# olegroshka/vae-channel-dynamics

Hardware: AMD Instinct MI355X
Metric: images/sec SDXL-VAE train step @256x256 (tracking on) (higher is better)
Workload: dtype f32

## Files before the change

### vae-channel-dynamics_amd/csrc/skinny.hip

```cpp
#include "thin_common.h"
#include "launchers.h"

#ifndef VAE_THIN_F32_MFMA
#define VAE_THIN_F32_MFMA 1
#endif

namespace {

using thin::TP;
using thin::TAPS_MAX;
constexpr int NT = 256;

__device__ __forceinline__ void stage_small(const vae_conv_geom& g, const float* __restrict__ S, int Cs_small, int K, int m0,
                                            int mrows, f32x4* __restrict__ sI) {
  const int hw = g.Ho * g.Wo;
  const size_t sbytes = (size_t)g.B * g.Hs * g.Ws * Cs_small * 4u;
  const auto rsS = VAE_BUF_RSRC(S, sbytes < BUF_MAX ? sbytes : BUF_MAX);
  for (int e = threadIdx.x; e < TP * g.taps; e += NT) {
    const int row = e / g.taps, tap = e - row * g.taps;
    const int m = m0 + row;
    const int b = m / hw, rem = m - b * hw;
    const int y = rem / g.Wo, x = rem - y * g.Wo;
    const int kh = (g.taps == 9) ? tap / 3 : 0, kw = (g.taps == 9) ? tap - kh * 3 : 0;
    int sy = 0, sx = 0;
    const bool ok = (m < mrows) && src_pixel(g, y, x, kh, kw, sy, sx);
    const unsigned base = ok ? (unsigned)(((b * g.Hs + sy) * g.Ws + sx) * Cs_small) * 4u : BUF_OOB;
    f32x4 v = {0.f, 0.f, 0.f, 0.f};
#pragma unroll
    for (int s = 0; s < 4; ++s)
      if (s < K) v[s] = __builtin_bit_cast(float, __builtin_amdgcn_raw_buffer_load_b32(rsS, ok ? base + 4u * s : BUF_OOB, 0, 0));
    sI[e] = v;
  }
}

__global__ __launch_bounds__(NT) void conv_smallk_kernel(vae_igemm_args p) {
  __shared__ f32x4 sI[TP * TAPS_MAX];
  const vae_conv_geom g = p.g;
  const int tid = threadIdx.x, lane = tid & 127, half = tid >> 7;
  const int m0 = blockIdx.x * TP;
  const int n = blockIdx.y * 128 + lane;
  const bool nok = n < p.N;
  stage_small(g, p.A, g.Cs, p.K, m0, p.M, sI);

  float w[TAPS_MAX][4];
#pragma unroll
  for (int t = 0; t < TAPS_MAX; ++t)
#pragma unroll
    for (int s = 0; s < 4; ++s)
      w[t][s] = (nok && t < g.taps && s < p.K) ? p.W[(int64_t)n * p.sn + (int64_t)t * p.st + (int64_t)s * p.sk] : 0.f;
  const float bv = (p.bias && nok) ? p.bias[n] : 0.f;
  const bool cbf = p.out_bf16 != 0;
  const size_t obytes = (size_t)p.M * p.ldc * (cbf ? 2u : 4u);
  const auto rsC = VAE_BUF_RSRC(p.C, obytes);
  __syncthreads();

  float tsum = 0.f;
#pragma unroll 4
  for (int i = 0; i < TP / 2; ++i) {
    const int row = half + 2 * i;
    float acc = bv;
#pragma unroll
    for (int t = 0; t < TAPS_MAX; ++t) {
      if (t < g.taps) {
        const f32x4 v = sI[row * g.taps + t];
#pragma unroll
        for (int s = 0; s < 4; ++s) acc += v[s] * w[t][s];
      }
    }
    const int m = m0 + row;
    const bool ok = nok && m < p.M;
    buf_store1_elem(rsC, cbf, ok ? m * p.ldc + n : -1, acc);
    const float stored = cbf ? (float)(__bf16)acc : acc;
    tsum += ok ? fabsf(stored) : 0.f;
  }
  if (p.track) {
    __syncthreads();
    float* red = reinterpret_cast<float*>(sI);
    red[tid] = tsum;
    __syncthreads();
    if (half == 0 && nok) p.track[(int64_t)blockIdx.x * p.N + n] = red[lane] + red[128 + lane];
  }
}

#if VAE_THIN_F32_MFMA
constexpr int WM_LDT = TP + 4;
constexpr int WM_ROWS = 48;
constexpr int WM_ITEMS = (TP * TAPS_MAX + NT - 1) / NT;
constexpr int WG_SI = WM_ROWS * WM_LDT / 4;
static_assert(WG_SI >= TP * TAPS_MAX + 32 && WG_SI >= NT, "LDS of wgrad_smallk_kernel");

template <bool SMALL_X, int XF>
__device__ __forceinline__ bool wgrad_mfma_serves(const vae_wgrad_args& p, const vae_conv_geom& gs) {
  const int wide = SMALL_X ? p.M : p.N, ldv = SMALL_X ? p.ldy : p.g.Cs;
  const bool vbf = (SMALL_X ? p.y_bf16 : p.x_bf16) != 0;
  const uintptr_t v = reinterpret_cast<uintptr_t>(SMALL_X ? p.dY : p.X);
  return gs.taps == TAPS_MAX && wide >= 64 && wide % 2 == 0 && ldv % 2 == 0 && (v & (vbf ? 3u : 7u)) == 0 &&
         (XF == VAE_XF_NONE || (gs.Ho * gs.Wo) % TP == 0);
}

template <bool SMALL_X, int XF>
__device__ __forceinline__ void wgrad_smallk_mfma(const vae_wgrad_args& p, const vae_conv_geom& gs, int ntiles, float* __restrict__ sT) {
  const int tid = threadIdx.x, lane = tid & 63, wave = tid >> 6;
  const int lc = lane & 15, lg = lane >> 4;
  const int split = blockIdx.x;
  const int wide = SMALL_X ? p.M : p.N, narrow = SMALL_X ? p.N : p.M;
  const int cq = blockIdx.y * 128 + wave * 32 + lc * 2;
  const float* __restrict__ V = SMALL_X ? p.dY : p.X;
  const float* __restrict__ S = SMALL_X ? p.X : p.dY;
  const int ldv = SMALL_X ? p.ldy : p.g.Cs, lds_ = SMALL_X ? p.g.Cs : p.ldy;
  const int npixv = gs.B * gs.Ho * gs.Wo, hwv = gs.Ho * gs.Wo;
  const bool vbf = (SMALL_X ? p.y_bf16 : p.x_bf16) != 0;
  const unsigned esV = vbf ? 2u : 4u;
  const size_t vbytes = (size_t)npixv * ldv * esV;
  const auto rsV = VAE_BUF_RSRC(V, vbytes < BUF_MAX ? vbytes : BUF_MAX);
  const auto rsS = thin::narrow_rsrc(S, gs, lds_);

  for (int i = tid; i < (WM_ROWS - 36) * WM_LDT; i += NT) sT[36 * WM_LDT + i] = (SMALL_X && i < WM_LDT) ? 1.f : 0.f;

  f32x4 acc[3][2];
#pragma unroll
  for (int mb = 0; mb < 3; ++mb)
#pragma unroll
    for (int e = 0; e < 2; ++e) acc[mb][e] = f32x4{0.f, 0.f, 0.f, 0.f};
  f32x4 ssum = {0.f, 0.f, 0.f, 0.f};
  float sc[2] = {0.f, 0.f}, sh[2] = {0.f, 0.f};
  int xb = -1;

  auto load_v = [&](uint2 (&rv)[8], int mb_) {
#pragma unroll
    for (int k = 0; k < 8; ++k) {
      const int m = mb_ + 16 * (k >> 2) + (k & 3);
      const int eoff = neg_unless(m < npixv && cq < wide, m * ldv + cq);
      rv[k] = __builtin_bit_cast(uint2, __builtin_amdgcn_raw_buffer_load_b64(rsV, eoff >= 0 ? (unsigned)eoff * esV : BUF_OOB, 0, 0));
    }
  };
  const int trow = tid & (TP - 1), thalf = __builtin_amdgcn_readfirstlane(tid >> 7);
  f32x4 rt[WM_ITEMS];
  auto load_t = [&](int tile, bool valid) {
    int m = tile * TP + trow;
    asm volatile("" : "+v"(m));
#pragma unroll
    for (int i = 0; i < WM_ITEMS; ++i) {
      const int tap = 2 * i + thalf;
      rt[i] = thin::gather4(gs, rsS, lds_, narrow, hwv, m, tap, valid && tap < TAPS_MAX && m < npixv);
    }
  };
  auto store_t = [&]() {
#pragma unroll
    for (int i = 0; i < WM_ITEMS; ++i) {
      const int tap = 2 * i + thalf;
      if (tap < TAPS_MAX) {
#pragma unroll
        for (int s = 0; s < 4; ++s) sT[(tap * 4 + s) * WM_LDT + trow] = rt[i][s];
        if (!SMALL_X && tap == TAPS_MAX / 2) ssum += rt[i];
      }
    }
  };
  auto chunk = [&](const uint2 (&rv)[8], int c) {
#pragma unroll
    for (int h = 0; h < 2; ++h) {
      f32x4 fa[3];
#pragma unroll
      for (int mb = 0; mb < 3; ++mb) fa[mb] = *reinterpret_cast<const f32x4*>(&sT[(mb * 16 + lc) * WM_LDT + c * 32 + h * 16 + 4 * lg]);
#pragma unroll
      for (int j = 0; j < 4; ++j) {
        const uint2 r = rv[h * 4 + j];
        float v[2];
        v[0] = __builtin_bit_cast(float, vbf ? r.x << 16 : r.x);
        v[1] = __builtin_bit_cast(float, vbf ? r.x & 0xffff0000u : r.y);
        if (XF != VAE_XF_NONE) {
#pragma unroll
          for (int e = 0; e < 2; ++e) v[e] = thin::xform1<XF>(v[e], sc[e], sh[e], cq + e < wide);
        }
#pragma unroll
        for (int mb = 0; mb < 3; ++mb)
#pragma unroll
          for (int e = 0; e < 2; ++e) acc[mb][e] = __builtin_amdgcn_mfma_f32_16x16x4f32(fa[mb][j], v[e], acc[mb][e], 0, 0, 0);
      }
    }
  };

  const thin::TileRange tr = thin::tile_range(split, thin::tiles_per_part(ntiles, p.nsplit), ntiles);
  const int pofs = 4 * lg;
  uint2 rva[8], rvb[8];
  if (tr.beg < tr.end) {
    load_t(tr.beg, true);
    load_v(rva, tr.beg * TP + pofs);
  }
  for (int tile = tr.beg; tile < tr.end; ++tile) {
    int mb0 = tile * TP + pofs;
    asm volatile("" : "+v"(mb0));
    const bool more = tile + 1 < tr.end;
    __syncthreads();
    store_t();
    __syncthreads();
    load_t(tile + 1, more);
    if (XF != VAE_XF_NONE) {
      const int b = (tile * TP) / hwv;
      if (b != xb) {
        xb = b;
#pragma unroll
        for (int e = 0; e < 2; ++e) {
          sc[e] = (cq + e < wide) ? p.scale[(int64_t)b * p.g.Cs + cq + e] : 0.f;
          sh[e] = (cq + e < wide) ? p.shift[(int64_t)b * p.g.Cs + cq + e] : 0.f;
        }
      }
    }
    load_v(rvb, mb0 + 32);
    chunk(rva, 0);
    load_v(rva, mb0 + 64);
    chunk(rvb, 1);
    load_v(rvb, mb0 + 96);
    chunk(rva, 2);
    load_v(rva, more ? mb0 + TP : npixv);
    chunk(rvb, 3);
  }

  const thin::Slab sl = thin::slab_of(p, split, TAPS_MAX);
#pragma unroll
  for (int mb = 0; mb < 3; ++mb)
#pragma unroll
    for (int e = 0; e < 2; ++e)
#pragma unroll
      for (int r = 0; r < 4; ++r) {
        const int t = mb * 4 + lg, ch = cq + e;
        if (ch < wide) {
          if (t < TAPS_MAX && r < narrow) thin::slab_store<SMALL_X>(sl, ch, t, r, acc[mb][e][r]);
          if (SMALL_X && mb == 2 && r == 0 && lg == 1 && p.bias_partial) thin::bias_partial_row(p, split)[ch] = acc[mb][e][r];
        }
      }
  if (!SMALL_X && p.bias_partial && blockIdx.y == 0) {
    __syncthreads();
#pragma unroll
    for (int s = 0; s < 4; ++s) sT[s * NT + tid] = ssum[s];
    __syncthreads();
    if (tid < p.M) {
      float t = 0.f;
      for (int i = 0; i < NT; ++i) t += sT[tid * NT + i];
      thin::bias_partial_row(p, split)[tid] = t;
    }
  }
}
#define WG_BOUNDS __launch_bounds__(NT, 4)
#else
constexpr int WG_SI = TP * TAPS_MAX + 32;
#define WG_BOUNDS __launch_bounds__(NT)
#endif

template <bool SMALL_X, int XF>
__global__ WG_BOUNDS void wgrad_smallk_kernel(vae_wgrad_args p, vae_conv_geom gs, int ntiles) {
  __shared__ f32x4 sI[WG_SI];
#if VAE_THIN_F32_MFMA
  if (wgrad_mfma_serves<SMALL_X, XF>(p, gs)) {
    wgrad_smallk_mfma<SMALL_X, XF>(p, gs, ntiles, reinterpret_cast<float*>(sI));
    return;
  }
#endif
  const int tid = threadIdx.x, lane = tid & 127, half = tid >> 7;
  const int split = blockIdx.x;
  const int ch = blockIdx.y * 128 + lane;
  const int wide = SMALL_X ? p.M : p.N, narrow = SMALL_X ? p.N : p.M;
  const bool chok = ch < wide;
  const float* __restrict__ V = SMALL_X ? p.dY : p.X;
  const float* __restrict__ S = SMALL_X ? p.X : p.dY;
  const int ldv = SMALL_X ? p.ldy : p.g.Cs, lds_ = SMALL_X ? p.g.Cs : p.ldy;
  const int npixv = gs.B * gs.Ho * gs.Wo;
  const int hwv = gs.Ho * gs.Wo;
  const bool vbf = (SMALL_X ? p.y_bf16 : p.x_bf16) != 0;
  const size_t vbytes = (size_t)npixv * ldv * (vbf ? 2u : 4u);
  const auto rsV = VAE_BUF_RSRC(V, vbytes < BUF_MAX ? vbytes : BUF_MAX);

  float acc[TAPS_MAX][4];
#pragma unroll
  for (int t = 0; t < TAPS_MAX; ++t)
#pragma unroll
    for (int s = 0; s < 4; ++s) acc[t][s] = 0.f;
  float vsum = 0.f;
  f32x4 ssum = {0.f, 0.f, 0.f, 0.f};
  int xb = -1;
  float xsc = 1.f, xsh = 0.f;

  const thin::TileRange tr = thin::tile_range(split, thin::tiles_per_part(ntiles, p.nsplit), ntiles);
  for (int tile = tr.beg; tile < tr.end; ++tile) {
    const int m0 = tile * TP;
    __syncthreads();
    stage_small(gs, S, lds_, narrow, m0, npixv, sI);
    __syncthreads();
#pragma unroll 4
    for (int i = 0; i < TP / 2; ++i) {
      const int row = half + 2 * i;
      const int m = m0 + row;
      const bool ok = chok && m < npixv;
      float v = buf_load1_elem(rsV, vbf, ok ? m * ldv + ch : -1);
      if (XF != VAE_XF_NONE) {
        const int b = min(m, npixv - 1) / hwv;
        if (b != xb) {
          xb = b;
          xsc = chok ? p.scale[(int64_t)b * p.g.Cs + ch] : 0.f;
          xsh = chok ? p.shift[(int64_t)b * p.g.Cs + ch] : 0.f;
        }
        v = thin::xform1<XF>(v, xsc, xsh, ok);
      }
      if (SMALL_X) vsum += v;
#pragma unroll
      for (int t = 0; t < TAPS_MAX; ++t) {
        if (t < gs.taps) {
          const f32x4 sv = sI[row * gs.taps + t];
#pragma unroll
          for (int s = 0; s < 4; ++s) acc[t][s] += v * sv[s];
          if (!SMALL_X && t == gs.taps / 2) ssum += sv;
        }
      }
    }
  }

  __syncthreads();
  float* red = reinterpret_cast<float*>(sI);
  if (half == 1) {
#pragma unroll
    for (int t = 0; t < TAPS_MAX; ++t)
#pragma unroll
      for (int s = 0; s < 4; ++s) red[lane * 36 + t * 4 + s] = acc[t][s];
    if (SMALL_X) red[128 * 36 + lane] = vsum;
    else if (lane == 0) {
#pragma unroll
      for (int s = 0; s < 4; ++s) red[128 * 36 + s] = ssum[s];
    }
  }
  __syncthreads();
  if (half == 0) {
    const thin::Slab sl = thin::slab_of(p, split, gs.taps);
    if (chok) {
#pragma unroll
      for (int t = 0; t < TAPS_MAX; ++t)
#pragma unroll
        for (int s = 0; s < 4; ++s)
          if (t < gs.taps && s < narrow) thin::slab_store<SMALL_X>(sl, ch, t, s, acc[t][s] + red[lane * 36 + t * 4 + s]);
    }
    if (p.bias_partial) {
      if (SMALL_X) {
        if (chok) thin::bias_partial_row(p, split)[ch] = vsum + red[128 * 36 + lane];
      } else if (blockIdx.y == 0 && lane < p.M) {
        thin::bias_partial_row(p, split)[lane] = ssum[lane] + red[128 * 36 + lane];
      }
    }
  }
}

}

bool conv_smallk_eligible(const vae_igemm_args& a) {
  const vae_conv_geom& g = a.g;
  return a.K <= 4 && a.batch == 1 && a.xf == VAE_XF_NONE && a.res == nullptr && a.alpha == 1.0f && g.taps <= TAPS_MAX &&
         g.mode != VAE_MODE_DGRAD_S2 && thin::desc_fits((size_t)a.M * a.ldc, 4u) && thin::narrow_fits(g);
}
int launch_conv_smallk(const vae_igemm_args& a, hipStream_t st) {
  dim3 grid((unsigned)((a.M + TP - 1) / TP), (unsigned)((a.N + 127) / 128));
  hipLaunchKernelGGL(conv_smallk_kernel, grid, dim3(NT), 0, st, a);
  return 0;
}

int wgrad_smallk_kind(const vae_wgrad_args& a) { return thin::wgrad_kind(a); }
int wgrad_smallk_tiles(const vae_wgrad_args& a) { return thin::wgrad_tiles(a); }

int launch_wgrad_smallk(const vae_wgrad_args& a, hipStream_t st) {
  const int kind = thin::wgrad_kind(a), ntiles = thin::wgrad_tiles(a);
  const vae_conv_geom gs = thin::wgrad_geom(a, kind);
  const dim3 grid = thin::wgrad_grid(a, kind);
  if (kind == 1) hipLaunchKernelGGL((wgrad_smallk_kernel<true, VAE_XF_NONE>), grid, dim3(NT), 0, st, a, gs, ntiles);
  else dispatch_xf_or_silu(a.xf, [&](auto xf) { hipLaunchKernelGGL((wgrad_smallk_kernel<false, decltype(xf)::value>), grid, dim3(NT), 0, st, a, gs, ntiles); });
  return 0;
}

namespace {

constexpr int NTH = thin::TH, NTW = thin::TW, NHW = thin::HW, NHP = thin::HP;
constexpr int NBK = 32, NLD = NBK + 4, NNT = 128;
constexpr int NHQ = NHP * (NBK / 4), NHI = (NHQ + NNT - 1) / NNT;

template <int XF>
__global__ __launch_bounds__(NNT) void conv_smalln_kernel(vae_igemm_args p, int tiles_x, int tiles_y) {
  __shared__ __attribute__((aligned(16))) float sH[NHP * NLD];
  const vae_conv_geom g = p.g;
  const int tid = threadIdx.x;
  const thin::Tile tl = thin::decode(blockIdx.x, tiles_x, tiles_y);
  const int b = tl.b, y0 = tl.y0, x0 = tl.x0;
  const int pr = tid >> 5, px = tid & 31;
  const bool abf = p.a_bf16 != 0;
  const unsigned esA = abf ? 2u : 4u;
  const auto rsA = VAE_BUF_RSRC(reinterpret_cast<const char*>(p.A) + (int64_t)b * g.Hs * g.Ws * g.Cs * esA, (size_t)g.Hs * g.Ws * g.Cs * esA);
  const float* __restrict__ W = p.W;

  float acc[4] = {0.f, 0.f, 0.f, 0.f};
  const int hk4 = tid & 7;
  uint4 rh[NHI];
  int hmask = 0;
  f32x4 rsc = {0.f, 0.f, 0.f, 0.f}, rsh = {0.f, 0.f, 0.f, 0.f};
  auto load_halo = [&](int c0) {
    hmask = 0;
    const int c = c0 + hk4 * 4;
    if (XF != VAE_XF_NONE) {
      const int cs = min(c, p.K - 4);
      rsc = *reinterpret_cast<const f32x4*>(p.scale + (int64_t)b * g.Cs + cs);
      rsh = *reinterpret_cast<const f32x4*>(p.shift + (int64_t)b * g.Cs + cs);
    }
#pragma unroll
    for (int i = 0; i < NHI; ++i) {
      const int q = tid + NNT * i;
      const int pp = q >> 3;
      const int ir = pp / NHW, jc = pp - ir * NHW;
      const int hy = y0 - 1 + ir, hx = x0 - 1 + jc;
      const bool ok = (q < NHQ) && ((unsigned)hy < (unsigned)g.Hs) && ((unsigned)hx < (unsigned)g.Ws) && (c < p.K);
      rh[i] = buf_load4_raw(rsA, esA, ok ? ((hy * g.Ws + hx) * g.Cs + c) : -1);
      hmask |= (ok ? 1 : 0) << i;
    }
  };
  auto store_halo = [&]() {
#pragma unroll
    for (int i = 0; i < NHI; ++i) {
      const int q = tid + NNT * i;
      if (q < NHQ) {
        f32x4 v = raw4_to_f32(rh[i], abf);
#pragma unroll
        for (int e = 0; e < 4; ++e) v[e] = thin::xform1<XF>(v[e], rsc[e], rsh[e], (hmask >> i) & 1);
        *reinterpret_cast<f32x4*>(&sH[(q >> 3) * NLD + hk4 * 4]) = v;
      }
    }
  };

  const int kchunks = (p.K + NBK - 1) / NBK;
  load_halo(0);
  for (int cch = 0; cch < kchunks; ++cch) {
    const int c0 = cch * NBK;
    __syncthreads();
    store_halo();
    __syncthreads();
    if (cch + 1 < kchunks) load_halo(c0 + NBK);
#pragma unroll
    for (int tap = 0; tap < 9; ++tap) {
      const int kh = tap / 3, kw = tap - kh * 3;
      const float* hrow = &sH[((pr + kh) * NHW + px + kw) * NLD];
#pragma unroll
      for (int q = 0; q < NBK / 4; ++q) {
        const f32x4 a = *reinterpret_cast<const f32x4*>(hrow + q * 4);
#pragma unroll
        for (int s = 0; s < 4; ++s) {
          if (s < p.N) {
            const f32x4 w4 = *reinterpret_cast<const f32x4*>(W + (int64_t)s * p.sn + (int64_t)tap * p.st + c0 + q * 4);
#pragma unroll
            for (int e = 0; e < 4; ++e) acc[s] = __builtin_fmaf(a[e], w4[e], acc[s]);
          }
        }
      }
    }
  }

  const int oy = y0 + pr, ox = x0 + px;
  const auto rsC = VAE_BUF_RSRC(p.C + (int64_t)b * g.Ho * g.Wo * p.ldc, (size_t)g.Ho * g.Wo * p.ldc * 4u);
#pragma unroll
  for (int s = 0; s < 4; ++s)
    if (s < p.N) {
      const float v = acc[s] + (p.bias ? p.bias[s] : 0.f);
      __builtin_amdgcn_raw_buffer_store_b32(__builtin_bit_cast(unsigned, v), rsC,
                                            (oy < g.Ho && ox < g.Wo) ? (unsigned)((oy * g.Wo + ox) * p.ldc + s) * 4u : BUF_OOB, 0, 0);
    }
}

}

bool conv_smalln_eligible(const vae_igemm_args& a) {
  const vae_conv_geom& g = a.g;
  return a.N <= 4 && a.K >= NBK && a.K % NBK == 0 && a.sn % 4 == 0 && a.st % 4 == 0 && aligned16(a.W) && a.batch == 1 && a.res == nullptr && a.track == nullptr && a.alpha == 1.0f &&
         a.A16 == nullptr && thin::fwd_same_3x3(g) && g.Wo % NTW == 0 && g.Ho % NTH == 0 && a.sk == 1 && g.Cs % 4 == 0 && aligned16(a.A) &&
         (a.xf == VAE_XF_NONE || (aligned16(a.scale) && aligned16(a.shift))) &&
         thin::desc_fits(thin::image_elems(g), 4u) && thin::desc_fits((size_t)g.Ho * g.Wo * a.ldc, 4u);
}
int launch_conv_smalln(const vae_igemm_args& a, hipStream_t st) {
  int tx, ty;
  const dim3 grid = thin::tile_grid(a.g, tx, ty);
  dispatch_xf_or_silu(a.xf, [&](auto xf) { hipLaunchKernelGGL((conv_smalln_kernel<decltype(xf)::value>), grid, dim3(NNT), 0, st, a, tx, ty); });
  return 0;
}
```

Before: 121.0.

## Add f32 MFMA paths for small-K and small-N thin convolutions

Adds matrix-core (MFMA 16x16x4 f32) code paths for the small-K convolution (the RGB input conv) and the small-N convolution (the output conv), each selected at runtime when its shape conditions hold. The small-K path becomes a persistent-style kernel that processes several tiles per workgroup and prefetches the next tile's gather into registers, which amortizes weight loads. The small-N path computes per-tap partial products for the halo with MFMA, then sums the 9 taps from shared memory. These replace scalar FMA loops but add more shared memory, register pressure and a larger block size for the small-N kernel.

```diff
diff --git a/vae-channel-dynamics_amd/csrc/skinny.hip b/vae-channel-dynamics_amd/csrc/skinny.hip
--- a/vae-channel-dynamics_amd/csrc/skinny.hip
+++ b/vae-channel-dynamics_amd/csrc/skinny.hip
@@ -33,8 +33,124 @@
   }
 }
 
-__global__ __launch_bounds__(NT) void conv_smallk_kernel(vae_igemm_args p) {
+#if VAE_THIN_F32_MFMA
+constexpr int CM_ITEMS = (TP * TAPS_MAX + NT - 1) / NT;
+typedef unsigned int u32x2 __attribute__((ext_vector_type(2)));
+
+__host__ __device__ __forceinline__ bool conv_mfma_serves(const vae_igemm_args& p) {
+  return p.g.taps == TAPS_MAX && p.N >= 64 && p.N % 4 == 0 && p.ldc % 4 == 0 &&
+         (reinterpret_cast<uintptr_t>(p.C) & (p.out_bf16 ? 7u : 15u)) == 0;
+}
+inline int conv_mfma_tiles_per_wg(int ntiles) { return std::max(1, std::min(8, ntiles / 1024)); }
+
+__device__ __forceinline__ void conv_smallk_mfma(const vae_igemm_args& p, f32x4* __restrict__ sI) {
+  const vae_conv_geom g = p.g;
+  const int tid = threadIdx.x, lane = tid & 63, wave = tid >> 6;
+  const int lc = lane & 15, lg = lane >> 4;
+  const int nw = blockIdx.y * 128 + wave * 32;
+  const int hw = g.Ho * g.Wo;
+  const auto rsS = thin::narrow_rsrc(p.A, g, g.Cs);
+  const bool cbf = p.out_bf16 != 0;
+  const unsigned esC = cbf ? 2u : 4u;
+  const auto rsC = VAE_BUF_RSRC(p.C, (size_t)p.M * p.ldc * esC);
+
+  float wa[2][TAPS_MAX];
+  f32x4 bv[2];
+#pragma unroll
+  for (int cb = 0; cb < 2; ++cb) {
+    const int na = nw + cb * 16 + lc, nd = nw + cb * 16 + 4 * lg;
+#pragma unroll
+    for (int t = 0; t < TAPS_MAX; ++t)
+      wa[cb][t] = (na < p.N && lg < p.K) ? p.W[(int64_t)na * p.sn + (int64_t)t * p.st + (int64_t)lg * p.sk] : 0.f;
+#pragma unroll
+    for (int r = 0; r < 4; ++r) bv[cb][r] = (p.bias && nd < p.N) ? p.bias[nd + r] : 0.f;
+  }
+
+  f32x4 rt[CM_ITEMS];
+  auto gather = [&](int tile, bool valid) {
+    const int m0 = tile * TP;
+#pragma unroll
+    for (int i = 0; i < CM_ITEMS; ++i) {
+      const int e = tid + NT * i;
+      const int row = e / TAPS_MAX, tap = e - row * TAPS_MAX;
+      rt[i] = thin::gather4(g, rsS, g.Cs, p.K, hw, m0 + row, tap, valid && e < TP * TAPS_MAX && m0 + row < p.M);
+    }
+  };
+
+  const int ntiles = (p.M + TP - 1) / TP;
+  const thin::TileRange tr = thin::tile_range(blockIdx.x, thin::tiles_per_part(ntiles, (int)gridDim.x), ntiles);
+  const float* __restrict__ sT = reinterpret_cast<const float*>(sI);
+  if (tr.beg < tr.end) gather(tr.beg, true);
+  for (int tile = tr.beg; tile < tr.end; ++tile) {
+    __syncthreads();
+#pragma unroll
+    for (int i = 0; i < CM_ITEMS; ++i) {
+      const int e = tid + NT * i;
+      if (e < TP * TAPS_MAX) sI[e] = rt[i];
+    }
+    __syncthreads();
+    gather(tile + 1, tile + 1 < tr.end);
+
+    f32x4 tsum[2] = {{0.f, 0.f, 0.f, 0.f}, {0.f, 0.f, 0.f, 0.f}};
+#pragma unroll 2
+    for (int pb = 0; pb < TP / 16; ++pb) {
+      const int prow = pb * 16 + lc;
+      f32x4 acc[2] = {bv[0], bv[1]};
+#pragma unroll
+      for (int t = 0; t < TAPS_MAX; ++t) {
+        const float b = sT[(prow * TAPS_MAX + t) * 4 + lg];
+#pragma unroll
+        for (int cb = 0; cb < 2; ++cb) acc[cb] = __builtin_amdgcn_mfma_f32_16x16x4f32(wa[cb][t], b, acc[cb], 0, 0, 0);
+      }
+      const int m = tile * TP + prow;
+#pragma unroll
+      for (int cb = 0; cb < 2; ++cb) {
+        const int nd = nw + cb * 16 + 4 * lg;
+        const bool ok = m < p.M && nd < p.N;
+        const int eoff = neg_unless(ok, m * p.ldc + nd);
+        const unsigned off = eoff >= 0 ? (unsigned)eoff * esC : BUF_OOB;
+        f32x4 stored = acc[cb];
+        if (cbf) {
+          const uint2 h = pack4(acc[cb]);
+          __builtin_amdgcn_raw_buffer_store_b64(u32x2{h.x, h.y}, rsC, off, 0, 0);
+          stored = unpack4(h);
+        } else {
+          __builtin_amdgcn_raw_buffer_store_b128(__builtin_bit_cast(u32x4, acc[cb]), rsC, off, 0, 0);
+        }
+#pragma unroll
+        for (int r = 0; r < 4; ++r) tsum[cb][r] += ok ? fabsf(stored[r]) : 0.f;
+      }
+    }
+    if (p.track) {
+#pragma unroll
+      for (int cb = 0; cb < 2; ++cb) {
+        const int nd = nw + cb * 16 + 4 * lg;
+#pragma unroll
+        for (int r = 0; r < 4; ++r) {
+          float v = tsum[cb][r];
+          v += lane_plus<8>(v);
+          v += lane_plus<4>(v);
+          v += lane_plus<2>(v);
+          v += lane_plus<1>(v);
+          if (lc == 0 && nd < p.N) p.track[(int64_t)tile * p.N + nd + r] = v;
+        }
+      }
+    }
+  }
+}
+#define CK_BOUNDS __launch_bounds__(NT, 4)
+#else
+#define CK_BOUNDS __launch_bounds__(NT)
+#endif
+
+__global__ CK_BOUNDS void conv_smallk_kernel(vae_igemm_args p) {
   __shared__ f32x4 sI[TP * TAPS_MAX];
+#if VAE_THIN_F32_MFMA
+  if (conv_mfma_serves(p)) {
+    conv_smallk_mfma(p, sI);
+    return;
+  }
+#endif
   const vae_conv_geom g = p.g;
   const int tid = threadIdx.x, lane = tid & 127, half = tid >> 7;
   const int m0 = blockIdx.x * TP;
@@ -355,6 +471,14 @@
          g.mode != VAE_MODE_DGRAD_S2 && thin::desc_fits((size_t)a.M * a.ldc, 4u) && thin::narrow_fits(g);
 }
 int launch_conv_smallk(const vae_igemm_args& a, hipStream_t st) {
+#if VAE_THIN_F32_MFMA
+  if (conv_mfma_serves(a)) {
+    const int ntiles = (a.M + TP - 1) / TP;
+    dim3 grid((unsigned)thin::tiles_per_part(ntiles, conv_mfma_tiles_per_wg(ntiles)), (unsigned)((a.N + 127) / 128));
+    hipLaunchKernelGGL(conv_smallk_kernel, grid, dim3(NT), 0, st, a);
+    return 0;
+  }
+#endif
   dim3 grid((unsigned)((a.M + TP - 1) / TP), (unsigned)((a.N + 127) / 128));
   hipLaunchKernelGGL(conv_smallk_kernel, grid, dim3(NT), 0, st, a);
   return 0;
@@ -378,9 +502,145 @@
 constexpr int NBK = 32, NLD = NBK + 4, NNT = 128;
 constexpr int NHQ = NHP * (NBK / 4), NHI = (NHQ + NNT - 1) / NNT;
 
+#if VAE_THIN_F32_MFMA
+constexpr int NM_NT = 256, NM_KMAX = 128;
+constexpr int NM_LDW = NM_KMAX + 4;
+constexpr int NM_ROWS = 9 * 4;
+constexpr int NM_CB = (NHP + 15) / 16;
+constexpr int NM_LDP = NM_CB * 16 + 4;
+constexpr int NM_LDS = NM_ROWS * NM_LDW + NM_ROWS * NM_LDP;
+constexpr int NSH = NM_LDS > NHP * NLD ? NM_LDS : NHP * NLD;
+
+__host__ __device__ __forceinline__ bool smalln_mfma_serves(const vae_igemm_args& p) { return p.K <= NM_KMAX; }
+
 template <int XF>
-__global__ __launch_bounds__(NNT) void conv_smalln_kernel(vae_igemm_args p, int tiles_x, int tiles_y) {
-  __shared__ __attribute__((aligned(16))) float sH[NHP * NLD];
+__device__ __forceinline__ void conv_smalln_mfma(const vae_igemm_args& p, int tiles_x, int tiles_y, float* __restrict__ sM) {
+  float* __restrict__ sW = sM;
+  float* __restrict__ sP = sM + NM_ROWS * NM_LDW;
+  const vae_conv_geom g = p.g;
+  const int tid = threadIdx.x, lane = tid & 63, wave = tid >> 6;
+  const int lc = lane & 15, lg = lane >> 4;
+  const thin::Tile tl = thin::decode(blockIdx.x, tiles_x, tiles_y);
+  const int b = tl.b, y0 = tl.y0, x0 = tl.x0;
+  const bool abf = p.a_bf16 != 0;
+  const unsigned esA = abf ? 2u : 4u;
+  const auto rsA = VAE_BUF_RSRC(reinterpret_cast<const char*>(p.A) + (int64_t)b * g.Hs * g.Ws * g.Cs * esA, (size_t)g.Hs * g.Ws * g.Cs * esA);
+  const int rows = 9 * p.N, rbn = (rows + 15) >> 4;
+  const int k4 = p.K >> 2;
+
+  for (int i = tid; i < NM_ROWS * k4; i += NM_NT) {
+    const int r = i / k4, c4 = i - r * k4;
+    const int tap = r / p.N, s = r - tap * p.N;
+    f32x4 w = {0.f, 0.f, 0.f, 0.f};
+    if (r < rows) w = *reinterpret_cast<const f32x4*>(p.W + (int64_t)s * p.sn + (int64_t)tap * p.st + c4 * 4);
+    *reinterpret_cast<f32x4*>(&sW[r * NM_LDW + c4 * 4]) = w;
+  }
+
+  int eo[4];
+#pragma unroll
+  for (int ci = 0; ci < 4; ++ci) {
+    const int q = (wave + 4 * ci) * 16 + lc;
+    const int ir = q / NHW, jc = q - ir * NHW;
+    const int hy = y0 - 1 + ir, hx = x0 - 1 + jc;
+    const bool ok = (q < NHP) && ((unsigned)hy < (unsigned)g.Hs) && ((unsigned)hx < (unsigned)g.Ws);
+    eo[ci] = neg_unless(ok, (hy * g.Ws + hx) * g.Cs);
+  }
+  const int ncb = wave == 0 ? 4 : 3;
+
+  f32x4 acc[4][3];
+#pragma unroll
+  for (int ci = 0; ci < 4; ++ci)
+#pragma unroll
+    for (int rb = 0; rb < 3; ++rb) acc[ci][rb] = f32x4{0.f, 0.f, 0.f, 0.f};
+
+  uint4 rx[2][4];
+  auto load_x = [&](int c0) {
+#pragma unroll
+    for (int j = 0; j < 2; ++j)
+#pragma unroll
+      for (int ci = 0; ci < 4; ++ci) rx[j][ci] = buf_load4_raw(rsA, esA, (eo[ci] >= 0 && ci < ncb) ? eo[ci] + c0 + 16 * j + 4 * lg : -1);
+  };
+  load_x(0);
+  __syncthreads();
+
+  for (int c0 = 0; c0 < p.K; c0 += NBK) {
+    uint4 cx[2][4];
+#pragma unroll
+    for (int j = 0; j < 2; ++j)
+#pragma unroll
+      for (int ci = 0; ci < 4; ++ci) cx[j][ci] = rx[j][ci];
+    f32x4 sc[2], sh[2];
+#pragma unroll
+    for (int j = 0; j < 2; ++j) {
+      sc[j] = sh[j] = f32x4{0.f, 0.f, 0.f, 0.f};
+      if (XF != VAE_XF_NONE) {
+        sc[j] = *reinterpret_cast<const f32x4*>(p.scale + (int64_t)b * g.Cs + c0 + 16 * j + 4 * lg);
+        sh[j] = *reinterpret_cast<const f32x4*>(p.shift + (int64_t)b * g.Cs + c0 + 16 * j + 4 * lg);
+      }
+    }
+    if (c0 + NBK < p.K) load_x(c0 + NBK);
+#pragma unroll
+    for (int j = 0; j < 2; ++j) {
+      f32x4 fa[3];
+#pragma unroll
+      for (int rb = 0; rb < 3; ++rb) fa[rb] = *reinterpret_cast<const f32x4*>(&sW[min(rb * 16 + lc, NM_ROWS - 1) * NM_LDW + c0 + 16 * j + 4 * lg]);
+#pragma unroll
+      for (int ci = 0; ci < 4; ++ci) {
+        if (ci < ncb) {
+          f32x4 v = raw4_to_f32(cx[j][ci], abf);
+#pragma unroll
+          for (int e = 0; e < 4; ++e) v[e] = thin::xform1<XF>(v[e], sc[j][e], sh[j][e], eo[ci] >= 0);
+#pragma unroll
+          for (int e = 0; e < 4; ++e)
+#pragma unroll
+            for (int rb = 0; rb < 3; ++rb)
+              if (rb < rbn) acc[ci][rb] = __builtin_amdgcn_mfma_f32_16x16x4f32(fa[rb][e], v[e], acc[ci][rb], 0, 0, 0);
+        }
+      }
+    }
+  }
+
+#pragma unroll
+  for (int ci = 0; ci < 4; ++ci)
+#pragma unroll
+    for (int rb = 0; rb < 3; ++rb)
+#pragma unroll
+      for (int r = 0; r < 4; ++r) {
+        const int row = rb * 16 + 4 * lg + r;
+        if (ci < ncb && row < rows) sP[row * NM_LDP + (wave + 4 * ci) * 16 + lc] = acc[ci][rb][r];
+      }
+  __syncthreads();
+
+  if (tid < NTH * NTW) {
+    const int pr = tid >> 5, px = tid & 31;
+    const int oy = y0 + pr, ox = x0 + px;
+    const auto rsC = VAE_BUF_RSRC(p.C + (int64_t)b * g.Ho * g.Wo * p.ldc, (size_t)g.Ho * g.Wo * p.ldc * 4u);
+#pragma unroll
+    for (int s = 0; s < 4; ++s)
+      if (s < p.N) {
+        float y = p.bias ? p.bias[s] : 0.f;
+#pragma unroll
+        for (int tap = 0; tap < 9; ++tap) y += sP[(tap * p.N + s) * NM_LDP + (pr + tap / 3) * NHW + px + tap % 3];
+        __builtin_amdgcn_raw_buffer_store_b32(__builtin_bit_cast(unsigned, y), rsC,
+                                              (oy < g.Ho && ox < g.Wo) ? (unsigned)((oy * g.Wo + ox) * p.ldc + s) * 4u : BUF_OOB, 0, 0);
+      }
+  }
+}
+#define CN_BOUNDS __launch_bounds__(NM_NT)
+#else
+constexpr int NSH = NHP * NLD;
+#define CN_BOUNDS __launch_bounds__(NNT)
+#endif
+
+template <int XF>
+__global__ CN_BOUNDS void conv_smalln_kernel(vae_igemm_args p, int tiles_x, int tiles_y) {
+  __shared__ __attribute__((aligned(16))) float sH[NSH];
+#if VAE_THIN_F32_MFMA
+  if (smalln_mfma_serves(p)) {
+    conv_smalln_mfma<XF>(p, tiles_x, tiles_y, sH);
+    return;
+  }
+#endif
   const vae_conv_geom g = p.g;
   const int tid = threadIdx.x;
   const thin::Tile tl = thin::decode(blockIdx.x, tiles_x, tiles_y);
@@ -478,6 +738,11 @@
 int launch_conv_smalln(const vae_igemm_args& a, hipStream_t st) {
   int tx, ty;
   const dim3 grid = thin::tile_grid(a.g, tx, ty);
-  dispatch_xf_or_silu(a.xf, [&](auto xf) { hipLaunchKernelGGL((conv_smalln_kernel<decltype(xf)::value>), grid, dim3(NNT), 0, st, a, tx, ty); });
+#if VAE_THIN_F32_MFMA
+  const int nt = smalln_mfma_serves(a) ? NM_NT : NNT;
+#else
+  const int nt = NNT;
+#endif
+  dispatch_xf_or_silu(a.xf, [&](auto xf) { hipLaunchKernelGGL((conv_smalln_kernel<decltype(xf)::value>), grid, dim3(nt), 0, st, a, tx, ty); });
   return 0;
 }
```

New measurement: 121.1 (median of 2 runs). About the same (+0.0%).

## Route small-K and small-N 3x3 convs through f32 MFMA kernels

Applied to the files above, without the earlier changes.

Adds an MFMA f32 16x16x4 path for the small-K (input-channel) conv kernel. It stages the im2col tile in LDS and computes 32 output channels per wave with vectorised stores and a shuffle-based tracking reduction. It also rewrites the small-N conv kernel as a 256-thread MFMA GEMM over halo pixels by 9*N tap-channel columns, double-buffering the halo and weights, then sums taps from LDS. This replaces scalar FMA loops with matrix-core work, at the cost of more LDS, a changed block size and wasted MFMA work on padded columns.

```diff
diff --git a/vae-channel-dynamics_amd/csrc/skinny.hip b/vae-channel-dynamics_amd/csrc/skinny.hip
--- a/vae-channel-dynamics_amd/csrc/skinny.hip
+++ b/vae-channel-dynamics_amd/csrc/skinny.hip
@@ -33,8 +33,130 @@
   }
 }
 
+#if VAE_THIN_F32_MFMA
+constexpr int WM_LDT = TP + 4;
+constexpr int WM_ROWS = 48;
+constexpr int WM_ITEMS = (TP * TAPS_MAX + NT - 1) / NT;
+__device__ __forceinline__ void t_gather(f32x4 (&rt)[WM_ITEMS], const vae_conv_geom& gs, __amdgpu_buffer_rsrc_t rsS, int lds_, int narrow,
+                                         int hwv, int npixv, int m, int thalf, bool valid) {
+#pragma unroll
+  for (int i = 0; i < WM_ITEMS; ++i) {
+    const int tap = 2 * i + thalf;
+    rt[i] = thin::gather4(gs, rsS, lds_, narrow, hwv, m, tap, valid && tap < TAPS_MAX && m < npixv);
+  }
+}
+__device__ __forceinline__ void t_store(const f32x4 (&rt)[WM_ITEMS], float* __restrict__ sT, int trow, int thalf) {
+#pragma unroll
+  for (int i = 0; i < WM_ITEMS; ++i) {
+    const int tap = 2 * i + thalf;
+    if (tap < TAPS_MAX) {
+#pragma unroll
+      for (int s = 0; s < 4; ++s) sT[(tap * 4 + s) * WM_LDT + trow] = rt[i][s];
+    }
+  }
+}
+
+__device__ __forceinline__ bool conv_mfma_serves(const vae_igemm_args& p) {
+  const bool cbf = p.out_bf16 != 0;
+  return p.g.taps == TAPS_MAX && p.g.stride == 1 && p.N >= 64 && p.N % 4 == 0 && p.ldc % 4 == 0 &&
+         (reinterpret_cast<uintptr_t>(p.C) & (cbf ? 7u : 15u)) == 0;
+}
+
+__device__ __forceinline__ void conv_smallk_mfma(const vae_igemm_args& p, float* __restrict__ sT) {
+  const vae_conv_geom& g = p.g;
+  const int tid = threadIdx.x, lane = tid & 63, wave = tid >> 6;
+  const int lc = lane & 15, lg = lane >> 4;
+  const int m0 = blockIdx.x * TP;
+  const int nb = blockIdx.y * 128 + wave * 32;
+
+  f32x4 rt[WM_ITEMS];
+  t_gather(rt, g, thin::narrow_rsrc(p.A, g, g.Cs), g.Cs, p.K, g.Ho * g.Wo, p.M, m0 + (tid & (TP - 1)), __builtin_amdgcn_readfirstlane(tid >> 7), true);
+
+  float a[TAPS_MAX][2];
+  f32x4 bv[2];
+#pragma unroll
+  for (int e = 0; e < 2; ++e) {
+    const int n = nb + 16 * e + lc;
+#pragma unroll
+    for (int t = 0; t < TAPS_MAX; ++t) a[t][e] = (n < p.N && lg < p.K) ? p.W[(int64_t)n * p.sn + (int64_t)t * p.st + (int64_t)lg * p.sk] : 0.f;
+#pragma unroll
+    for (int r = 0; r < 4; ++r) {
+      const int nr = nb + 16 * e + 4 * lg + r;
+      bv[e][r] = (p.bias && nr < p.N) ? p.bias[nr] : 0.f;
+    }
+  }
+  const bool cbf = p.out_bf16 != 0;
+  const unsigned esC = cbf ? 2u : 4u;
+  const auto rsC = VAE_BUF_RSRC(p.C, (size_t)p.M * p.ldc * esC);
+
+  t_store(rt, sT, tid & (TP - 1), __builtin_amdgcn_readfirstlane(tid >> 7));
+  __syncthreads();
+
+  f32x4 tsum[2] = {f32x4{0.f, 0.f, 0.f, 0.f}, f32x4{0.f, 0.f, 0.f, 0.f}};
+#pragma unroll
+  for (int c = 0; c < TP / 64; ++c) {
+    f32x4 acc[4][2];
+#pragma unroll
+    for (int q = 0; q < 4; ++q)
+#pragma unroll
+      for (int e = 0; e < 2; ++e) acc[q][e] = bv[e];
+#pragma unroll
+    for (int t = 0; t < TAPS_MAX; ++t) {
+      const f32x4 b = *reinterpret_cast<const f32x4*>(&sT[(t * 4 + lg) * WM_LDT + c * 64 + 4 * lc]);
+#pragma unroll
+      for (int q = 0; q < 4; ++q)
+#pragma unroll
+        for (int e = 0; e < 2; ++e) acc[q][e] = __builtin_amdgcn_mfma_f32_16x16x4f32(a[t][e], b[q], acc[q][e], 0, 0, 0);
+    }
+#pragma unroll
+    for (int q = 0; q < 4; ++q) {
+      const int m = m0 + c * 64 + 4 * lc + q;
+#pragma unroll
+      for (int e = 0; e < 2; ++e) {
+        const int n = nb + 16 * e + 4 * lg;
+        const bool ok = m < p.M && n < p.N;
+        const unsigned off = oob_unless(ok, (unsigned)(m * p.ldc + n) * esC);
+        f32x4 stored = acc[q][e];
+        if (cbf) {
+          const uint2 h = pack4(stored);
+          typedef unsigned int u32x2 __attribute__((ext_vector_type(2)));
+          __builtin_amdgcn_raw_buffer_store_b64(__builtin_bit_cast(u32x2, h), rsC, off, 0, 0);
+          stored = unpack4(h);
+        } else {
+          __builtin_amdgcn_raw_buffer_store_b128(__builtin_bit_cast(u32x4, stored), rsC, off, 0, 0);
+        }
+#pragma unroll
+        for (int r = 0; r < 4; ++r) tsum[e][r] += ok ? fabsf(stored[r]) : 0.f;
+      }
+    }
+  }
+  if (p.track) {
+#pragma unroll
+    for (int e = 0; e < 2; ++e)
+#pragma unroll
+      for (int r = 0; r < 4; ++r) {
+        float v = tsum[e][r];
+#pragma unroll
+        for (int d = 1; d < 16; d *= 2) v += __shfl_xor(v, d, 64);
+        const int n = nb + 16 * e + 4 * lg + r;
+        if (lc == 0 && n < p.N) p.track[(int64_t)blockIdx.x * p.N + n] = v;
+      }
+  }
+}
+constexpr int SK_SI = TAPS_MAX * 4 * WM_LDT / 4;
+#else
+constexpr int SK_SI = TP * TAPS_MAX;
+#endif
+static_assert(SK_SI >= TP * TAPS_MAX, "LDS of conv_smallk_kernel");
+
 __global__ __launch_bounds__(NT) void conv_smallk_kernel(vae_igemm_args p) {
-  __shared__ f32x4 sI[TP * TAPS_MAX];
+  __shared__ f32x4 sI[SK_SI];
+#if VAE_THIN_F32_MFMA
+  if (conv_mfma_serves(p)) {
+    conv_smallk_mfma(p, reinterpret_cast<float*>(sI));
+    return;
+  }
+#endif
   const vae_conv_geom g = p.g;
   const int tid = threadIdx.x, lane = tid & 127, half = tid >> 7;
   const int m0 = blockIdx.x * TP;
@@ -83,9 +205,6 @@
 }
 
 #if VAE_THIN_F32_MFMA
-constexpr int WM_LDT = TP + 4;
-constexpr int WM_ROWS = 48;
-constexpr int WM_ITEMS = (TP * TAPS_MAX + NT - 1) / NT;
 constexpr int WG_SI = WM_ROWS * WM_LDT / 4;
 static_assert(WG_SI >= TP * TAPS_MAX + 32 && WG_SI >= NT, "LDS of wgrad_smallk_kernel");
 
@@ -139,11 +258,7 @@
   auto load_t = [&](int tile, bool valid) {
     int m = tile * TP + trow;
     asm volatile("" : "+v"(m));
-#pragma unroll
-    for (int i = 0; i < WM_ITEMS; ++i) {
-      const int tap = 2 * i + thalf;
-      rt[i] = thin::gather4(gs, rsS, lds_, narrow, hwv, m, tap, valid && tap < TAPS_MAX && m < npixv);
-    }
+    t_gather(rt, gs, rsS, lds_, narrow, hwv, npixv, m, thalf, valid);
   };
   auto store_t = [&]() {
 #pragma unroll
@@ -375,8 +490,169 @@
 namespace {
 
 constexpr int NTH = thin::TH, NTW = thin::TW, NHW = thin::HW, NHP = thin::HP;
-constexpr int NBK = 32, NLD = NBK + 4, NNT = 128;
-constexpr int NHQ = NHP * (NBK / 4), NHI = (NHQ + NNT - 1) / NNT;
+constexpr int NBK = 32, NLD = NBK + 4;
+constexpr int NHQ = NHP * (NBK / 4);
+
+#if VAE_THIN_F32_MFMA
+template <int XF, int NTHR>
+struct HaloStage {
+  static constexpr int NI = (NHQ + NTHR - 1) / NTHR;
+  uint4 rh[NI];
+  int hmask = 0;
+  f32x4 rsc = {0.f, 0.f, 0.f, 0.f}, rsh = {0.f, 0.f, 0.f, 0.f};
+  __device__ __forceinline__ void load(const vae_igemm_args& p, __amdgpu_buffer_rsrc_t rsA, unsigned esA, int b, int y0, int x0, int c0) {
+    const vae_conv_geom& g = p.g;
+    const int tid = threadIdx.x;
+    hmask = 0;
+    const int c = c0 + (tid & 7) * 4;
+    if (XF != VAE_XF_NONE) {
+      const int cs = min(c, p.K - 4);
+      rsc = *reinterpret_cast<const f32x4*>(p.scale + (int64_t)b * g.Cs + cs);
+      rsh = *reinterpret_cast<const f32x4*>(p.shift + (int64_t)b * g.Cs + cs);
+    }
+#pragma unroll
+    for (int i = 0; i < NI; ++i) {
+      const int q = tid + NTHR * i;
+      const int pp = q >> 3;
+      const int ir = pp / NHW, jc = pp - ir * NHW;
+      const int hy = y0 - 1 + ir, hx = x0 - 1 + jc;
+      const bool ok = (q < NHQ) && ((unsigned)hy < (unsigned)g.Hs) && ((unsigned)hx < (unsigned)g.Ws) && (c < p.K);
+      rh[i] = buf_load4_raw(rsA, esA, ok ? ((hy * g.Ws + hx) * g.Cs + c) : -1);
+      hmask |= (ok ? 1 : 0) << i;
+    }
+  }
+  __device__ __forceinline__ void store(float* __restrict__ sH, bool abf) const {
+    const int tid = threadIdx.x;
+#pragma unroll
+    for (int i = 0; i < NI; ++i) {
+      const int q = tid + NTHR * i;
+      if (q < NHQ) {
+        f32x4 v = raw4_to_f32(rh[i], abf);
+#pragma unroll
+        for (int e = 0; e < 4; ++e) v[e] = thin::xform1<XF>(v[e], rsc[e], rsh[e], (hmask >> i) & 1);
+        *reinterpret_cast<f32x4*>(&sH[(q >> 3) * NLD + (tid & 7) * 4]) = v;
+      }
+    }
+  }
+};
+
+constexpr int NNT = 256;
+constexpr int NMB = (NHP + 15) / 16, NHR = NMB * 16;
+constexpr int NLP = NHR + 4;
+constexpr int NWF = 2 * 3 * 64;
+constexpr int NSM = NHR * NLD + NWF * 4;
+static_assert(NSM >= 36 * NLP, "P lies over the halo and the weights");
+
+template <int XF, int NB>
+__device__ __forceinline__ void conv_smalln_mfma(const vae_igemm_args& p, int tiles_x, int tiles_y, float* __restrict__ sH) {
+  constexpr int NIT = NMB * NB, IPW = (NIT + 3) / 4;
+  constexpr int NWI = (2 * NB * 64 + NNT - 1) / NNT;
+  f32x4* __restrict__ sW = reinterpret_cast<f32x4*>(sH + NHR * NLD);
+  const vae_conv_geom& g = p.g;
+  const int tid = threadIdx.x, lane = tid & 63, wave = __builtin_amdgcn_readfirstlane(tid >> 6);
+  const int lc = lane & 15, lg = lane >> 4;
+  const thin::Tile tl = thin::decode(blockIdx.x, tiles_x, tiles_y);
+  const int b = tl.b, y0 = tl.y0, x0 = tl.x0;
+  const bool abf = p.a_bf16 != 0;
+  const unsigned esA = abf ? 2u : 4u;
+  const auto rsA = VAE_BUF_RSRC(reinterpret_cast<const char*>(p.A) + (int64_t)b * g.Hs * g.Ws * g.Cs * esA, (size_t)g.Hs * g.Ws * g.Cs * esA);
+
+  const float* wsrc[NWI];
+  bool wok[NWI];
+#pragma unroll
+  for (int i = 0; i < NWI; ++i) {
+    const int f = tid + NNT * i, ln = f & 63, hn = f >> 6;
+    const int col = 16 * (hn % NB) + (ln & 15), tap = col / p.N, s = col - tap * p.N;
+    wok[i] = f < 2 * NB * 64 && col < 9 * p.N;
+    wsrc[i] = p.W + (wok[i] ? (int64_t)s * p.sn + (int64_t)tap * p.st + 16 * (hn / NB) + 4 * (ln >> 4) : 0);
+  }
+  f32x4 rw[NWI];
+  auto load_w = [&](int c0) {
+#pragma unroll
+    for (int i = 0; i < NWI; ++i) rw[i] = wok[i] ? *reinterpret_cast<const f32x4*>(wsrc[i] + c0) : f32x4{0.f, 0.f, 0.f, 0.f};
+  };
+  auto store_w = [&]() {
+#pragma unroll
+    for (int i = 0; i < NWI; ++i)
+      if (tid + NNT * i < 2 * NB * 64) sW[tid + NNT * i] = rw[i];
+  };
+
+  f32x4 acc[IPW];
+#pragma unroll
+  for (int i = 0; i < IPW; ++i) acc[i] = f32x4{0.f, 0.f, 0.f, 0.f};
+  int aofs[IPW], bofs[IPW];
+#pragma unroll
+  for (int i = 0; i < IPW; ++i) {
+    const int it = min(wave * IPW + i, NIT - 1);
+    const int nb = it / NMB, mb = it - nb * NMB;
+    aofs[i] = (16 * mb + lc) * NLD + 4 * lg;
+    bofs[i] = nb * 64 + lane;
+  }
+
+  HaloStage<XF, NNT> hs;
+  const int kchunks = p.K / NBK;
+  hs.load(p, rsA, esA, b, y0, x0, 0);
+  load_w(0);
+  for (int cch = 0; cch < kchunks; ++cch) {
+    __syncthreads();
+    hs.store(sH, abf);
+    store_w();
+    __syncthreads();
+    if (cch + 1 < kchunks) {
+      hs.load(p, rsA, esA, b, y0, x0, (cch + 1) * NBK);
+      load_w((cch + 1) * NBK);
+    }
+#pragma unroll
+    for (int h = 0; h < 2; ++h)
+#pragma unroll
+      for (int i0 = 0; i0 < IPW; i0 += 4) {
+        f32x4 fa[4], fb[4];
+#pragma unroll
+        for (int i = i0; i < IPW && i < i0 + 4; ++i) {
+          fa[i - i0] = *reinterpret_cast<const f32x4*>(&sH[aofs[i] + 16 * h]);
+          fb[i - i0] = sW[bofs[i] + h * NB * 64];
+        }
+#pragma unroll
+        for (int j = 0; j < 4; ++j)
+#pragma unroll
+          for (int i = i0; i < IPW && i < i0 + 4; ++i) acc[i] = __builtin_amdgcn_mfma_f32_16x16x4f32(fa[i - i0][j], fb[i - i0][j], acc[i], 0, 0, 0);
+      }
+  }
+
+  __syncthreads();
+  float* __restrict__ sP = sH;
+#pragma unroll
+  for (int i = 0; i < IPW; ++i) {
+    const int it = wave * IPW + i;
+    const int nb = it / NMB, mb = it - nb * NMB, col = 16 * nb + lc;
+    if (it < NIT && col < 9 * p.N) *reinterpret_cast<f32x4*>(&sP[col * NLP + 16 * mb + 4 * lg]) = acc[i];
+  }
+  __syncthreads();
+  const auto rsC = VAE_BUF_RSRC(p.C + (int64_t)b * g.Ho * g.Wo * p.ldc, (size_t)g.Ho * g.Wo * p.ldc * 4u);
+#pragma unroll
+  for (int k = 0; k < NTH * NTW * 4 / NNT; ++k) {
+    const int o = tid + NNT * k, pix = o & (NTH * NTW - 1), s = o / (NTH * NTW);
+    if (s < p.N) {
+      const int pr = pix / NTW, px = pix - pr * NTW;
+      float v = p.bias ? p.bias[s] : 0.f;
+#pragma unroll
+      for (int tap = 0; tap < 9; ++tap) v += sP[(tap * p.N + s) * NLP + (pr + tap / 3) * NHW + px + tap % 3];
+      const int oy = y0 + pr, ox = x0 + px;
+      __builtin_amdgcn_raw_buffer_store_b32(__builtin_bit_cast(unsigned, v), rsC,
+                                            (oy < g.Ho && ox < g.Wo) ? (unsigned)((oy * g.Wo + ox) * p.ldc + s) * 4u : BUF_OOB, 0, 0);
+    }
+  }
+}
+
+template <int XF>
+__global__ __launch_bounds__(NNT, 3) void conv_smalln_kernel(vae_igemm_args p, int tiles_x, int tiles_y) {
+  __shared__ __attribute__((aligned(16))) float sH[NSM];
+  if (p.N <= 3) conv_smalln_mfma<XF, 2>(p, tiles_x, tiles_y, sH);
+  else conv_smalln_mfma<XF, 3>(p, tiles_x, tiles_y, sH);
+}
+#else
+constexpr int NNT = 128;
+constexpr int NHI = (NHQ + NNT - 1) / NNT;
 
 template <int XF>
 __global__ __launch_bounds__(NNT) void conv_smalln_kernel(vae_igemm_args p, int tiles_x, int tiles_y) {
@@ -465,6 +741,7 @@
                                             (oy < g.Ho && ox < g.Wo) ? (unsigned)((oy * g.Wo + ox) * p.ldc + s) * 4u : BUF_OOB, 0, 0);
     }
 }
+#endif
 
 }
 
```

After: 118.1 before, 118.4 after (median of 6 runs). About the same (+0.3%).
